# alexisvannson/GraphNet_Classifier

Hardware: AMD Instinct MI355X
Metric: edges aggregated/sec (GraphNet forward) (higher is better)
Workload: dtype f32; 1 GPU; c3: 1M nodes / 10M edges (6250 graphs x 160 nodes x 1600 edges), D=64, 2 GN blocks; graphs=6250, nodes=1000000, edges=10000000, n_blocks=2, width=64, step=CSR build + GraphNet.forward, inputs resident in HBM

## Files before the change

graphnet_classifier_amd/csrc/mlp_device.h:

```cpp
#pragma once
#include "gnc_common.h"

namespace gnc_mlp {

typedef float f32x16 __attribute__((ext_vector_type(16)));
typedef float f32x4 __attribute__((ext_vector_type(4)));

constexpr int KC = 64;
constexpr int LDSW = 68;
constexpr int RPW = 32;

__device__ __forceinline__ f32x16 mfma(float a, float b, f32x16 c) {
  return __builtin_amdgcn_mfma_f32_32x32x2f32(a, b, c, 0, 0, 0);
}

__device__ __forceinline__ void wave_lds_fence() {
  asm volatile("s_waitcnt lgkmcnt(0)" ::: "memory");
}

__device__ __forceinline__ float activate(float x, int act, float p) {
  switch (act) {
    case GNC_ACT_RELU: return x < 0.f ? 0.f : x;
    case GNC_ACT_IDENTITY: return x;
    case GNC_ACT_TANH: return tanhf(x);
// ... 933 lines not shown

struct BwdArgs {
  const float* grad_out;
  int ld_grad_out;
  float* act[GNC_MAX_LINEAR];
  float* dz[GNC_MAX_LINEAR];
  float* dx;
  int ld_dx;
  float* yhat;
  int dx_add_grad_out;
  float* ln_partial;
  const float* gg;
  const int* gg_index;
  int ld_gg;
  int64_t gg_rows;
  float* g_sum;
  int ld_g_sum;
};

__host__ __device__ inline int ldw_of(const gnc_mlp_desc_t& d, int l) { return d.ld_weight[l] ? d.ld_weight[l] : d.in_dim[l]; }

inline bool al16(const void* p) { return (reinterpret_cast<uintptr_t>(p) & 15u) == 0; }

inline int tiles_for(int width) {
  const int t = (width + 31) / 32;
  return t <= 1 ? 1 : t <= 2 ? 2 : t <= 4 ? 4 : 8;
}

int validate_desc(const gnc_mlp_desc_t* d, bool check_ptrs);
int launch_resident_dual(const float* x, int64_t ld_x, int64_t rows, const float* wa, int64_t ld_wa, const float* wb, int64_t ld_wb,
                         int in_dim, int out_dim, float* out_a, float* out_b, int64_t ld_out, hipStream_t stream, bool* launched);
int launch_resident(const gnc_mlp_desc_t& d, int T, bool narrow_out, hipStream_t stream, bool* launched,
                    bool probe_only = false, bool agg_only = false);
int launch_stream(const gnc_mlp_desc_t& d, int T, bool narrow_out, hipStream_t stream, bool* launched,
                  bool probe_only = false);
int launch_stream16(const gnc_mlp_desc_t& d, hipStream_t stream, bool* launched, bool probe_only = false);
int launch_col16(const gnc_mlp_desc_t& d, hipStream_t stream, bool* launched, bool probe_only = false);
int64_t col16_max_rows();
int64_t bwd_col16_max_rows();
bool bwd_col16_supported(const gnc_mlp_desc_t& d);
int bwd_col16_ln_partial_rows(int64_t rows);
int launch_bwd_col16(const gnc_mlp_bwd_desc_t& bd, hipStream_t stream);
bool bwd_col16_persist_supported(const gnc_mlp_desc_t& d);
int bwd_col16_persist_ln_partial_rows(int64_t rows);
int launch_bwd_col16_persist(const gnc_mlp_bwd_desc_t& bd, hipStream_t stream);
bool bwd_stream16_supported(const gnc_mlp_desc_t& d, bool want_dx);
int bwd_stream16_ln_partial_rows(int64_t rows);
int launch_bwd_stream16(const gnc_mlp_desc_t& d, const BwdArgs& b, hipStream_t stream, bool saved = false);

}
```

graphnet_classifier_amd/csrc/mlp_fused.hip:

```cpp
#include <stdlib.h>

#include "mlp_device.h"

using namespace gnc_mlp;

namespace {

constexpr int WAVES = 4;
constexpr int NT = WAVES * 64;
constexpr int RPB = RPW * WAVES;

__device__ __forceinline__ void stage_rows(float* abuf, const gnc_mlp_segment_t& seg, int64_t row0, int64_t rows,
                                           int c0, int ncol4, bool vec_ok, int lane) {
  const int c4 = lane & 15;
  const int rs = lane >> 4;
  if (c4 < ncol4) {
#pragma unroll
    for (int p = 0; p < RPW / 4; ++p) {
      const int j = p * 4 + rs;
      const int64_t r = row0 + j;
      f32x4 v = {0.f, 0.f, 0.f, 0.f};
      if (r < rows) {
        const int64_t tr = seg.index ? (int64_t)seg.index[r] : r;
        if (!seg.index || (uint64_t)tr < (uint64_t)seg.table_rows)
// ... 276 lines not shown
  if (rc) return rc;
  const auto [T, narrow_out] = tile_class(*desc);
  const gnc_mlp_desc_t probe = agg_probe(*desc);
  bool ok = false;
  {
    gnc_mlp_desc_t plain = *desc;
    plain.agg_out = nullptr;
    bool small = false;
    rc = launch_col16(plain, nullptr, &small, true);
    if (rc) return rc;
    if (small) {
      gnc::set_error("gnc_mlp_agg_supported: a small batch: run gnc_scatter_sum_csr_f32 on the output rows");
      return GNC_ERR_UNSUPPORTED;
    }
  }
  rc = launch_resident(probe, T, narrow_out, nullptr, &ok, true);
  if (rc) return rc;
  if (!ok && T == 4) {
    rc = launch_stream(probe, T, narrow_out, nullptr, &ok, true);
    if (rc) return rc;
  }
  if (!ok && T == 8) {
    rc = launch_stream16(probe, nullptr, &ok, true);
    if (rc) return rc;
  }
  if (!ok) {
    gnc::set_error("gnc_mlp_agg_supported: needs the weights-resident W-split shape (1 MATMUL + 2 ADD segments, residual = "
                   "the MATMUL segment, widths 33..64) or a 65..128-wide description of the streaming kernel");
    return GNC_ERR_UNSUPPORTED;
  }
  return GNC_OK;
}

extern "C" int gnc_mlp_agg_only_supported(const gnc_mlp_desc_t* desc) {
  int rc = gnc_mlp_agg_supported(desc);
  if (rc) return rc;
  const auto [T, narrow_out] = tile_class(*desc);
  const gnc_mlp_desc_t probe = agg_probe(*desc);
  bool ok = false;
  rc = launch_resident(probe, T, narrow_out, nullptr, &ok, true, true);
  if (rc) return rc;
  if (!ok) {
    gnc::set_error("gnc_mlp_agg_only_supported: needs the 64-wide W-split edge processor (1 MATMUL + 2 ADD segments, residual = "
                   "the MATMUL segment, three Linear layers, LayerNorm) without save_act");
    return GNC_ERR_UNSUPPORTED;
  }
  return GNC_OK;
}

extern "C" int gnc_mlp_forward_agg_only_f32(const gnc_mlp_desc_t* desc, void* stream) {
  int rc = validate_desc(desc, true);
  if (rc) return rc;
  if (!desc->agg_out || !desc->agg_index || !desc->agg_fix) {
    gnc::set_error("gnc_mlp_forward_agg_only_f32: agg_out, agg_index and agg_fix are required");
    return GNC_ERR_INVALID_ARGUMENT;
  }
  rc = gnc_mlp_agg_only_supported(desc);
  if (rc) return rc;
  if (desc->rows == 0) return GNC_OK;
  const auto [T, narrow_out] = tile_class(*desc);
  bool launched = false;
  rc = launch_resident(*desc, T, narrow_out, (hipStream_t)stream, &launched, false, true);
  if (!rc && !launched) {
    gnc::set_error("gnc_mlp_forward_agg_only_f32: the weights-resident kernel did not take the launch");
    rc = GNC_ERR_UNSUPPORTED;
  }
// ... 107 lines not shown
```

graphnet_classifier_amd/csrc/mlp_resident.hip:

```cpp
#include <stdlib.h>

#include "mlp_device.h"

using namespace gnc_mlp;

#ifdef GNC_PHASE_PROBE
__device__ unsigned long long gnc_phase_probe[4096 * 12];
extern "C" int gnc_phase_probe_read(void* dst, size_t bytes) {
  return (int)hipMemcpyFromSymbol(dst, HIP_SYMBOL(gnc_phase_probe), bytes);
}
#define PROBE_BEGIN() unsigned long long pr_acc[8] = {0, 0, 0, 0, 0, 0, 0, 0}, pr_tp, pr_tn; \
  const unsigned long long pr_c0 = __builtin_readcyclecounter(), pr_w0 = wall_clock64()
#define PROBE_TILE() pr_tp = __builtin_readcyclecounter()
#define PROBE(k) do { pr_tn = __builtin_readcyclecounter(); pr_acc[k] += pr_tn - pr_tp; pr_tp = pr_tn; } while (0)
#define PROBE_END() do { if ((threadIdx.x & 63) == 0) {                                                      \
    unsigned long long* o = gnc_phase_probe + (blockIdx.x * (blockDim.x >> 6) + (threadIdx.x >> 6)) * 12;    \
    for (int k = 0; k < 8; ++k) o[k] = pr_acc[k];                                                            \
    o[8] = __builtin_readcyclecounter() - pr_c0; o[9] = wall_clock64() - pr_w0; } } while (0)
#else
#define PROBE_BEGIN() do {} while (0)
#define PROBE_TILE() do {} while (0)
#define PROBE(k) do {} while (0)
#define PROBE_END() do {} while (0)
#endif

namespace {

constexpr int RWAVES = 8;
constexpr int RNT = RWAVES * 64;

template <int HT, int OT, int NMM, int NADD, bool RESREG, bool AGG = false, bool SAVE = false, bool FULL = false, int EF = 0, bool DUAL = false,
          int SPLIT = 0, bool AGGONLY = false>
__global__ __launch_bounds__(RNT) void mlp_resident_kernel(const gnc_mlp_desc_t d, const int num_wtiles,
                                                           const int total_chunks) {
  extern __shared__ __attribute__((aligned(16))) float lds[];
  constexpr int WT = HT > OT ? HT : OT;
  constexpr int CH = WT * 32 * LDSW;
  static_assert(!FULL || OT == 2, "fixed widths: 64 out");
  static_assert(!FULL || NADD == 2 || (NMM == 1 && !RESREG && !AGG && !SAVE && !DUAL), "fixed-width plain stacks");
  constexpr int SEGW = EF != 0 ? 3 : KC;
  constexpr bool W32 = FULL && !SAVE;
  constexpr bool GADD = W32 && NADD == 2;
  static_assert(SPLIT == 0 || (HT == 2 && SPLIT == 1 && NMM == 1 && ((NADD == 2 && RESREG && !DUAL) || (NADD == 0 && !RESREG))) ||
                    (HT == 2 && OT == 2 && SPLIT == 2 && NADD == 0 && !DUAL),
                "split shapes");
  constexpr int nf32 = SPLIT == 1 ? 0 : NMM;
  constexpr bool SPK = !(SPLIT == 1 && NADD == 2 && AGG && !FULL && !SAVE);
  constexpr bool PIPE = SPLIT != 0 && SPK && !DUAL && (FULL || (SPLIT == 2 && NMM == 1) || (SPLIT == 1 && NADD == 0));
  constexpr bool FRONT = GADD && SPLIT == 1 && PIPE;
  constexpr int GPK = FRONT ? 4 : 2;
  __bf16* const wsp = reinterpret_cast<__bf16*>(lds + nf32 * CH);
  auto wsplit = [&](int chunk) -> const __bf16* { return wsp + (chunk - nf32) * 3 * SPLANE; };
  constexpr int PSTRIDE = WT * 32;
  constexpr int NS = NMM + NADD;
  const int tid = threadIdx.x;
  const int lane = tid & 63;
  const int wave = __builtin_amdgcn_readfirstlane(tid >> 6);
  const int i = lane & 31;
  const int h = lane >> 5;
  const int c4 = lane & 15;
  const int rs = lane >> 4;
  const int L = FULL ? 3 : d.num_linear;
  const int out_dim = FULL ? KC : d.out_dim[L - 1];
  const int rows = (int)d.rows;
  float* wres = lds;
  float* pbuf = SPLIT == 0 ? lds + total_chunks * CH : lds + nf32 * CH + (total_chunks - nf32) * SCH;
  float* abuf = pbuf + (L + 2) * PSTRIDE + wave * RPW * LDSW;

  stage_params<RNT>(pbuf, d, PSTRIDE, tid);
  if constexpr (SPLIT != 0) {
    const int ldw0 = ldw_of(d, 0);
    const bool w0v = (ldw0 % 4 == 0) && ((reinterpret_cast<uintptr_t>(d.weight[0]) & 15u) == 0);
    if constexpr (SPLIT == 1) {
      stage_weights_split<RNT>(wsp, d.weight[0], ldw0, d.out_dim[0], d.seg[0].wcol, d.seg[0].wcol + d.seg[0].width,
                               w0v && (d.seg[0].wcol % 4 == 0), tid);
    } else {
#pragma unroll
      for (int s = 0; s < NMM; ++s)
        stage_weights<WT * 32, RNT>(wres + s * CH, d.weight[0], ldw0, d.out_dim[0], d.seg[s].wcol, d.seg[s].wcol + d.seg[s].width, 16,
                                    w0v && (d.seg[s].wcol % 4 == 0), tid);
// ... 54 lines not shown
    const int col = c4 * 4 < s.ld ? c4 * 4 : 0;
    if (s.index == nullptr) {
      if constexpr (W32)
        load_tile_rows_w(pre, table_window(s.ptr, rows, s.ld), s.ld, (wt < num_wtiles ? wt : num_wtiles) * RPW, rows, (uint32_t)(rs * s.ld + col) * 4u);
      else load_tile_rows(pre, s.ptr, s.ld, (int64_t)wt * RPW, rows, (uint32_t)(rs * s.ld + col) * 4u);
    } else {
      const __amdgpu_buffer_rsrc_t w = __builtin_amdgcn_make_buffer_rsrc(const_cast<float*>(s.ptr), 0, (int)s.bytes, 0x00020000);
      const uint32_t row_bytes = off * (uint32_t)(s.ld * 4);
#pragma unroll
      for (int p = 0; p < NP; ++p) pre[p] = window_load(w, (uint32_t)__shfl((int)row_bytes, p * 4 + rs, 64) + (uint32_t)(col * 4));
    }
  };
  auto stage = [&](const f32x4 (&pre)[NP], int width) {
    compiler_lds_barrier();
    const int c = c4 * 4;
    if (width >= KC) {
#pragma unroll
      for (int p = 0; p < NP; ++p) *reinterpret_cast<f32x4*>(abuf + (p * 4 + rs) * LDSW + c) = pre[p];
    } else {
#pragma unroll
      for (int p = 0; p < NP; ++p) {
        f32x4 v = pre[p];
        v.x = c + 0 < width ? v.x : 0.f; v.y = c + 1 < width ? v.y : 0.f;
        v.z = c + 2 < width ? v.z : 0.f; v.w = c + 3 < width ? v.w : 0.f;
        *reinterpret_cast<f32x4*>(abuf + (p * 4 + rs) * LDSW + c) = v;
      }
    }
    compiler_lds_barrier();
  };

  const int gwave = (int)blockIdx.x * RWAVES + wave;
  const int stride = AGG ? 1 : total_waves;
  int wt = gwave, wt_end = num_wtiles;
  if constexpr (AGG) {
    const int q = num_wtiles / total_waves, rem = num_wtiles - q * total_waves;
    wt = gwave * q + (gwave < rem ? gwave : rem);
    wt_end = wt + q + (gwave < rem ? 1 : 0);
  }
  f32x4 cur[NP];
  f32x4 addA[NADD ? NP : 1], addB[NADD ? NP : 1];
  uint32_t offs[NS];
  typedef float f32x2 __attribute__((ext_vector_type(2)));
  int ef_s = 0, ef_d = 0;
  f32x2 ef_ps = {0.f, 0.f}, ef_pd = {0.f, 0.f};
  const __amdgpu_buffer_rsrc_t ef_win =
      __builtin_amdgcn_make_buffer_rsrc(const_cast<float*>(EF == 1 ? d.ef_pos : nullptr), 0, EF == 1 ? (int)(uint32_t)(d.ef_nodes * 8) : 0, 0x00020000);
  auto ef_ids = [&](int t) {
    const int tc = t < last_wt ? t : last_wt;
    int r = tc * RPW + (lane & 31);
    r = r < rows ? r : rows - 1;
    ef_s = d.ef_src[r];
    ef_d = d.ef_dst[r];
  };
  auto ef_fetch = [&]() {
    typedef uint32_t u32x2 __attribute__((ext_vector_type(2)));
    ef_ps = __builtin_bit_cast(f32x2, (u32x2)__builtin_amdgcn_raw_buffer_load_b64(ef_win, (uint32_t)ef_s * 8u, 0, 0));
    ef_pd = __builtin_bit_cast(f32x2, (u32x2)__builtin_amdgcn_raw_buffer_load_b64(ef_win, (uint32_t)ef_d * 8u, 0, 0));
  };
  auto ef_stage = [&]() {
    compiler_lds_barrier();
    const float dx = ef_pd.x - ef_ps.x, dy = ef_pd.y - ef_ps.y;
    f32x4 v = {dx, dy, __builtin_fabsf(dx) + __builtin_fabsf(dy), 0.f};
    if (h) v = f32x4{0.f, 0.f, 0.f, 0.f};
    *reinterpret_cast<f32x4*>(abuf + i * LDSW + 4 * h) = v;
    compiler_lds_barrier();
  };
  typedef float f32x3 __attribute__((ext_vector_type(3)));
  f32x3 n3_row = {0.f, 0.f, 0.f};
  const __amdgpu_buffer_rsrc_t n3_win = __builtin_amdgcn_make_buffer_rsrc(
      const_cast<float*>(EF == 2 ? d.seg[0].ptr : nullptr), 0, EF == 2 ? (int)(uint32_t)(d.rows * 12) : 0, 0x00020000);
// ... 9 lines not shown
    *reinterpret_cast<f32x4*>(abuf + i * LDSW + 4 * h) = v;
    compiler_lds_barrier();
  };
  uint32_t off0 = 0;
  if constexpr (EF == 1) {
    ef_ids(wt);
    ef_fetch();
    ef_ids(wt + stride);
  } else if constexpr (EF == 2) {
    n3_fetch(wt);
  } else {
    load_rows(cur, sv[0], wt, row_offset(wt, sv[0]));
  }
#pragma unroll
  for (int s = 1; s < NS; ++s) offs[s] = row_offset(wt, sv[s]);
  if constexpr (EF == 0) off0 = row_offset(wt + stride, sv[0]);

  const int col_out = c4 * 4;
  const bool vec_out = FULL || ((out_dim % 4 == 0) && (d.ld_out % 4 == 0) && ((reinterpret_cast<uintptr_t>(d.out) & 15u) == 0));
  const uint32_t out_lane_off = (uint32_t)(rs * d.ld_out + col_out) * 4u;
  const uint32_t res_lane_off = (uint32_t)(rs * d.ld_residual + (col_out < d.ld_residual ? col_out : 0)) * 4u;

  auto agg_ids = [&](int t) -> int {
    int r = t * RPW + (lane & 31);
    r = r < rows ? r : rows - 1;
    return d.agg_index[r];
  };
  int aid = 0, aid_next = 0;
  float agg_acc = 0.f;
  int agg_cur = -1, agg_first_dst = -1;
  bool agg_first = true;
  if constexpr (AGG) aid = agg_ids(wt < last_wt ? wt : last_wt);
  static_assert(!AGGONLY || (AGG && FULL && !SAVE && !DUAL), "aggregate-only: the FULL AGG inference instance");
  int keep_lo = -1, keep_hi = -1;
  if constexpr (AGGONLY) {
    if (wt < wt_end) {
      const int last_row = wt_end * RPW < rows ? wt_end * RPW - 1 : rows - 1;
      keep_lo = d.agg_index[wt * RPW];
      keep_hi = d.agg_index[last_row];
    }
  }
  uint32_t keep_rows = 0;

  PROBE_BEGIN();
  while (wt < wt_end) {
    PROBE_TILE();
    const int row0 = wt * RPW;
    const int nwt = wt + stride;
    if constexpr (AGG) aid_next = agg_ids(nwt < last_wt ? nwt : last_wt);

    f32x16 hid[HT];
    f32x16 res[RESREG ? HT : 1];
    init_bias<HT>(hid, pbuf, h);
#pragma unroll
    for (int s = 0; s < NMM; ++s) {
      bool interleaved = false;
      if constexpr (EF == 1) ef_stage();
      else if constexpr (EF == 2) n3_stage();
      else stage(cur, sv[s].width);
      PROBE(0);
      if (s + 1 < NMM) {
        load_rows(cur, sv[s + 1 < NMM ? s + 1 : 0], wt, offs[s + 1 < NMM ? s + 1 : 0]);
        offs[s + 1 < NMM ? s + 1 : 0] = row_offset(nwt, sv[s + 1 < NMM ? s + 1 : 0]);
      } else {
        if constexpr (NADD > 0) {
          if (GADD || (sv[s].width == KC && sv[NMM].index && sv[NMM + 1].index)) {
            const SegView &sa = sv[NMM], &sb = sv[NMM + 1];
            const __amdgpu_buffer_rsrc_t wa = __builtin_amdgcn_make_buffer_rsrc(const_cast<float*>(sa.ptr), 0, (int)sa.bytes, 0x00020000);
            const __amdgpu_buffer_rsrc_t wb = __builtin_amdgcn_make_buffer_rsrc(const_cast<float*>(sb.ptr), 0, (int)sb.bytes, 0x00020000);
            const uint32_t cola = (uint32_t)(c4 * 4 < sa.ld ? c4 * 16 : 0), colb = (uint32_t)(c4 * 4 < sb.ld ? c4 * 16 : 0);
            const int rba = (int)(offs[NMM] * (uint32_t)(sa.ld * 4)), rbb = (int)(offs[NMM + 1] * (uint32_t)(sb.ld * 4));
            int na = __shfl(rba, rs, 64), nb = __shfl(rbb, rs, 64);
            if constexpr (SPLIT == 1) {
              const __bf16* wch = wsplit(s);
              auto request = [&](int kg) {
#pragma unroll
                for (int g = GPK * kg; g < GPK * kg + GPK && g < 8; ++g) {
                  const uint32_t oa = (uint32_t)na + cola, ob = (uint32_t)nb + colb;
                  if (g + 1 < 8) {
                    na = __shfl(rba, (g + 1) * 4 + rs, 64);
                    nb = __shfl(rbb, (g + 1) * 4 + rs, 64);
// ... 158 lines not shown
      f32x16 o[OT];
      init_bias<OT>(o, pbuf + (L - 1) * PSTRIDE, h);
      if constexpr (PIPE) mma_chunk_from_regs_split_pipe<HT, OT, 4>(o, hid, wsplit(NMM + L - 2), i, h);
      else if constexpr (SPLIT != 0) mma_chunk_from_regs_split<HT, OT, SPK>(o, hid, wsplit(NMM + L - 2), FULL ? KC : d.in_dim[L - 1], i, h);
      else mma_chunk_from_regs<HT, OT>(o, hid, wres + (NMM + L - 2) * CH, 0, FULL ? KC : d.in_dim[L - 1], i, h);
      PROBE(4);
      if (FULL || d.ln_gamma) layer_norm_tiles<OT>(o, pbuf + L * PSTRIDE, pbuf + (L + 1) * PSTRIDE, out_dim, d.ln_eps, h);
      if constexpr (RESREG) {
#pragma unroll
        for (int t = 0; t < OT && t < HT; ++t) o[t] += res[t < HT ? t : 0];
      }
      compiler_lds_barrier();
      tiles_to_lds<OT>(o, abuf, i, h);
      PROBE(5);
    }
    compiler_lds_barrier();
    if constexpr (AGG) {
      const int valid = rows - row0 < RPW ? rows - row0 : RPW;
      int prv = __shfl_up(aid, 1, 64);
      prv = lane == 0 ? agg_cur : prv;
      const unsigned long long vmask = valid >= 32 ? 0xffffffffull : ((1ull << valid) - 1ull);
      const unsigned long long bnd = __ballot(aid != prv) & vmask;
      if constexpr (AGGONLY) keep_rows = (uint32_t)(__ballot(aid == keep_lo || aid == keep_hi) & vmask);
      float rowv[RPW];
#pragma unroll
      for (int r = 0; r < RPW; ++r) rowv[r] = abuf[r * LDSW + lane];
      auto agg_row = [&](int r) {
        if ((bnd >> r) & 1ull) {
          if (agg_cur >= 0) {
            if (agg_first) {
              agg_first = false;
              agg_first_dst = agg_cur;
            } else if (lane < out_dim) {
              float* dstp = d.agg_out + (int64_t)agg_cur * d.ld_agg;
              asm volatile("s_nop 4\n\tglobal_store_dword %0, %1, %2\n\ts_nop 0" ::"v"(lane * 4), "v"(agg_acc), "s"(dstp) : "memory");
            }
          }
          agg_cur = __builtin_amdgcn_readlane(aid, r);
          agg_acc = 0.f;
        }
        agg_acc += rowv[r];
      };
#pragma unroll
      for (int r4 = 0; r4 < RPW; r4 += 4) {
        if (r4 + 4 <= valid && ((bnd >> r4) & 0xfull) == 0) {
          agg_acc += rowv[r4 + 0];
          agg_acc += rowv[r4 + 1];
          agg_acc += rowv[r4 + 2];
          agg_acc += rowv[r4 + 3];
        } else {
#pragma unroll
          for (int r = r4; r < r4 + 4; ++r)
            if (r < valid) agg_row(r);
        }
      }
      aid = aid_next;
    }
    if constexpr (EF == 1) {
      asm volatile("" ::"v"(ef_ps), "v"(ef_pd), "v"(ef_s), "v"(ef_d));
    } else if constexpr (EF == 2) {
      asm volatile("" ::"v"(n3_row.x), "v"(n3_row.y), "v"(n3_row.z));
    } else {
#pragma unroll
      for (int p = 0; p < NP; ++p) asm volatile("" ::"v"(cur[p]));
    }
#pragma unroll
    for (int s = 1; s < NS; ++s) asm volatile("" ::"v"(offs[s]));
    asm volatile("" ::"v"(off0));
    if constexpr (AGG) asm volatile("" ::"v"(aid_next));

    if constexpr (AGGONLY) {
      if (keep_rows) {
#pragma unroll
        for (int p = 0; p < NP; ++p) {
          const f32x4 v = *reinterpret_cast<const f32x4*>(abuf + (p * 4 + rs) * LDSW + col_out);
          if ((keep_rows >> (p * 4 + rs)) & 1u)
            hidden_window_store<true>(v, out_lane_off + (uint32_t)(row0 + 4 * p) * (uint32_t)(d.ld_out * 4), table_window(d.out, rows, d.ld_out));
        }
      }
    } else {
      f32x4 outv[NP];
#pragma unroll
      for (int p = 0; p < NP; ++p) outv[p] = *reinterpret_cast<const f32x4*>(abuf + (p * 4 + rs) * LDSW + col_out);
      if ((!FULL || NADD != 0) && !RESREG && d.residual) {
        f32x4 rv[NP];
        load_tile_rows(rv, d.residual, d.ld_residual, row0, rows, res_lane_off);
#pragma unroll
        for (int p = 0; p < NP; ++p) outv[p] += rv[p];
      }
      if constexpr (W32) {
        store_tile_rows_w<true>(outv, table_window(d.out, rows, d.ld_out), d.ld_out, row0, rows, out_lane_off);
      } else if (vec_out) {
        if (col_out < out_dim) {
          if (row0 + RPW <= rows) {
            uint32_t r0b;
            const __amdgpu_buffer_rsrc_t ow = full_tile_window(d.out, row0, rows, d.ld_out, &r0b);
#pragma unroll
            for (int p = 0; p < NP; ++p) hidden_window_store_s<true>(outv[p], out_lane_off + r0b, ow, (uint32_t)(p * 16 * d.ld_out));
          } else {
#pragma unroll
            for (int p = 0; p < NP; ++p) hidden_window_store(outv[p], out_lane_off, row_window(d.out, row0 + 4 * p, rows, d.ld_out));
          }
        }
      } else {
#pragma unroll
        for (int p = 0; p < NP; ++p) {
          const int r = row0 + p * 4 + rs;
          store_row_piece(d.out + (int64_t)(r < rows ? r : rows - 1) * d.ld_out, col_out, outv[p], r < rows && col_out < out_dim,
                          out_dim, false);
        }
      }
    }
    if constexpr (DUAL) {
      compiler_lds_barrier();
      tiles_to_lds<HT>(hidb, abuf, i, h);
      compiler_lds_barrier();
      f32x4 outb[NP];
#pragma unroll
      for (int p = 0; p < NP; ++p) outb[p] = *reinterpret_cast<const f32x4*>(abuf + (p * 4 + rs) * LDSW + col_out);
      if (col_out < out_dim) {
        if (row0 + RPW <= rows) {
          uint32_t r0b;
          const __amdgpu_buffer_rsrc_t ow = full_tile_window(d.save_act[0], row0, rows, d.ld_out, &r0b);
#pragma unroll
          for (int p = 0; p < NP; ++p) hidden_window_store_s<true>(outb[p], out_lane_off + r0b, ow, (uint32_t)(p * 16 * d.ld_out));
        } else {
#pragma unroll
          for (int p = 0; p < NP; ++p) hidden_window_store(outb[p], out_lane_off, row_window(d.save_act[0], row0 + 4 * p, rows, d.ld_out));
        }
      }
    }
    compiler_lds_barrier();
    PROBE(6);
    wt = nwt;
  }
  if constexpr (AGG) {
    if (lane == 0) {
      d.agg_fix[2 * gwave] = agg_first ? agg_cur : agg_first_dst;
      d.agg_fix[2 * gwave + 1] = agg_cur;
    }
  }
  PROBE_END();
}

template <int HT, int OT, int NMM, int NADD, bool RESREG, bool AGG = false, bool SAVE = false, bool FULL = false, int EF = 0, bool DUAL = false,
          int SPLIT = 0, bool AGGONLY = false>
int launch(const gnc_mlp_desc_t& d, int total_chunks, size_t smem, hipStream_t stream) {
  void (*const kernel)(const gnc_mlp_desc_t, const int, const int) = &mlp_resident_kernel<HT, OT, NMM, NADD, RESREG, AGG, SAVE, FULL, EF, DUAL, SPLIT, AGGONLY>;
  static bool attr_set = false;
  if (!attr_set) {
    int rc = gnc::check_hip(hipFuncSetAttribute(reinterpret_cast<const void*>(kernel), hipFuncAttributeMaxDynamicSharedMemorySize, 160 * 1024),
                            "hipFuncSetAttribute(MaxDynamicSharedMemorySize)");
    if (rc) return rc;
    attr_set = true;
  }
  const int64_t num_wtiles = gnc::ceil_div(d.rows, RPW);
  int64_t grid = gnc::ceil_div(num_wtiles, RWAVES);
  if (grid > gnc::num_cu()) grid = gnc::num_cu();
  if constexpr (AGG) grid = gnc::num_cu();
  kernel<<<dim3((unsigned)grid), dim3(RNT), smem, stream>>>(d, (int)num_wtiles, total_chunks);
  return gnc::check_launch("mlp_resident_kernel");
}

template <int HT, int OT, int NMM, int NADD, bool RESREG, bool AGG = false, bool SAVE = false, bool FULL = false, int EF = 0,
          bool AGGONLY = false>
int launch_cls(int split, const gnc_mlp_desc_t& d, int total_chunks, size_t smem, hipStream_t stream) {
  if constexpr (HT == 2 && OT == 2 && NMM == 1 && NADD == 2 && RESREG) {
    if (split == 1) return launch<HT, OT, NMM, NADD, RESREG, AGG, SAVE, FULL, EF, false, 1, AGGONLY>(d, total_chunks, smem, stream);
  }
  if constexpr (HT == 2 && NMM == 1 && NADD == 0 && !RESREG && !AGG && !SAVE && !FULL && EF == 0) {
    if (split == 1) return launch<HT, OT, NMM, NADD, RESREG, AGG, SAVE, FULL, EF, false, 1>(d, total_chunks, smem, stream);
  }
  if constexpr (HT == 2 && OT == 2 && NADD == 0 && !AGG && (!FULL || EF != 0) && ((NMM == 1 && !RESREG) || (NMM == 2 && EF == 0))) {
    if (split == 2) return launch<HT, OT, NMM, NADD, RESREG, AGG, SAVE, FULL, EF, false, 2>(d, total_chunks, smem, stream);
  }
  if (split) return GNC_ERR_UNSUPPORTED;
  return launch<HT, OT, NMM, NADD, RESREG, AGG, SAVE, FULL, EF, false, 0, AGGONLY>(d, total_chunks, smem, stream);
}

}

static bool f32_exact() {
  static const bool v = getenv("GNC_MLP_F32_EXACT") != nullptr;
  return v;
}

extern "C" int gnc_mlp_agg_fix_len(void) { return 2 * gnc::num_cu() * RWAVES; }

int gnc_mlp::launch_resident_dual(const float* x, int64_t ld_x, int64_t rows, const float* wa, int64_t ld_wa, const float* wb,
                                  int64_t ld_wb, int in_dim, int out_dim, float* out_a, float* out_b, int64_t ld_out,
                                  hipStream_t stream, bool* launched) {
  *launched = false;
  static const bool disabled = getenv("GNC_MLP_NO_RESIDENT") != nullptr;
  if (disabled || rows < 1 || rows >= INT32_MAX || in_dim < 1 || in_dim > KC || out_dim <= 32 || out_dim > KC || out_dim % 4 != 0 ||
      ld_x % 4 != 0 || ld_x < in_dim || ld_out % 4 != 0 || ld_out < out_dim || ld_wa < in_dim || ld_wb < in_dim || ld_wa > INT32_MAX ||
      ld_wb > INT32_MAX || ld_x > INT32_MAX || ld_out > INT32_MAX || !al16(x) || !al16(out_a) || !al16(out_b))
    return GNC_OK;
  gnc_mlp_desc_t d = {};
  d.num_segments = 1;
  d.num_linear = 1;
  d.activation = GNC_ACT_RELU;
  d.seg[0].ptr = x;
  d.seg[0].width = in_dim;
  d.seg[0].ld = (int32_t)ld_x;
  d.seg[0].mode = GNC_SEG_MATMUL;
  d.weight[0] = wa;
  d.ld_weight[0] = (int32_t)ld_wa;
  d.weight[1] = wb;
  d.ld_weight[1] = (int32_t)ld_wb;
  d.in_dim[0] = in_dim;
  d.out_dim[0] = out_dim;
  d.in_dim[1] = in_dim;
  d.out = out_a;
  d.save_act[0] = out_b;
  d.ld_out = (int32_t)ld_out;
  d.rows = rows;
  const int total_chunks = 2;
  const bool split = !f32_exact();
  const size_t floats = (size_t)total_chunks * (split ? SCH : 2 * 32 * LDSW) + (size_t)(1 + 2) * 2 * 32 + (size_t)RWAVES * RPW * LDSW;
  *launched = true;
// ... 162 lines not shown
```

graphnet_classifier_amd/native.py:

```python
from __future__ import annotations

import ctypes
import math
import os
from ctypes import POINTER, Structure, c_char_p, c_double, c_float, c_int32, c_int64, c_size_t, c_void_p

import torch

LIB_NAME = "libgnc_hip.so"
LIB_PATH = os.path.join(os.path.dirname(os.path.abspath(__file__)), LIB_NAME)

GNC_MAX_SEGMENTS = 4
GNC_MAX_LINEAR = 8
ABI_VERSION = 20

ACTIVATIONS = {
    "ReLU": 0, "Identity": 1, "Tanh": 2, "Sigmoid": 3, "SiLU": 4, "GELU": 5, "LeakyReLU": 6, "ELU": 7,
}

_SIGNATURES = {
    "gnc_abi_version": (c_int32, []),
    "gnc_last_error_string": (c_char_p, []),
    "gnc_target_arch": (c_char_p, []),
    "gnc_mlp_agg_supported": (c_int32, [c_void_p]),
    "gnc_mlp_agg_only_supported": (c_int32, [c_void_p]),
    "gnc_mlp_forward_agg_only_f32": (c_int32, [c_void_p, c_void_p]),
    "gnc_mlp_edge_features_supported": (c_int32, [c_void_p]),
    "gnc_mlp_operands_in_place_supported": (c_int32, [c_void_p]),
    "gnc_mlp_save_act_supported": (c_int32, [c_void_p]),
    "gnc_mlp_agg_fix_len": (c_int32, []),
    "gnc_mlp_small_batch_supported": (c_int32, [c_void_p]),
    "gnc_mlp_small_batch_max_rows": (c_int64, []),
    "gnc_mlp_projection_t2_f32": (c_int32, [c_void_p, c_int64, c_void_p, c_int64, c_int64, c_void_p, c_int64, c_int32, c_int32, c_void_p,
                                            c_int64, c_void_p]),
    "gnc_mlp_dual_projection_f32": (c_int32, [c_void_p, c_int64, c_int64, c_void_p, c_int64, c_void_p, c_int64, c_int32, c_int32,
                                              c_void_p, c_void_p, c_int64, c_void_p]),
    "gnc_mlp_backward_small_batch_supported": (c_int32, [c_void_p]),
    "gnc_readout_forward_f32": (c_int32, [c_void_p, c_int64, c_void_p, c_int64, c_void_p, c_int32, c_void_p, c_int64, c_void_p, c_int32,
                                          c_void_p, c_int64, c_void_p, c_int32, c_void_p, c_void_p, c_void_p, c_void_p, c_void_p]),
    "gnc_readout_backward_f32": (c_int32, [c_void_p, c_void_p, c_int64, c_void_p, c_int64, c_int32, c_void_p, c_int64, c_int32, c_void_p,
                                           c_int64, c_int32, c_void_p, c_void_p, c_void_p, c_void_p, c_void_p, c_void_p, c_void_p, c_void_p,
                                           c_void_p, c_void_p]),
    "gnc_readout_batched_supported": (c_int32, [c_int64, c_int64, c_int32, c_int32, c_int32, c_void_p]),
    "gnc_readout_batched_forward_f32": (c_int32, [c_void_p, c_void_p, c_int64, c_int64, c_int32, c_int64, c_void_p, c_int64, c_void_p,
                                                  c_int32, c_void_p, c_int64, c_void_p, c_int32, c_void_p, c_int64, c_void_p, c_int32,
                                                  c_void_p, c_void_p, c_void_p, c_void_p, c_int64, c_void_p]),
    "gnc_readout_batched_backward_f32": (c_int32, [c_void_p, c_void_p, c_void_p, c_int64, c_int64, c_int32, c_int64, c_void_p, c_int64,
                                                   c_int32, c_void_p, c_int64, c_int32, c_void_p, c_int64, c_int32, c_void_p, c_void_p,
                                                   c_void_p, c_void_p, c_void_p, c_void_p, c_int64, c_void_p]),
    "gnc_pad_graph_batch_supported": (c_int32, [c_int64, c_int64, c_int64, c_int64, c_int64, c_int32, c_int32]),
    "gnc_pad_graph_batch": (c_int32, [c_void_p, c_int32, c_void_p, c_int32, c_void_p, c_int64, c_int64, c_int64, c_int64, c_void_p, c_void_p,
                                      c_void_p, c_int64, c_int64, c_void_p, c_void_p, c_void_p, c_void_p, c_void_p, c_void_p, c_void_p]),
    "gnc_xty_small_max_rows": (c_int32, []),
    "gnc_xty_small_f32": (c_int32, [c_void_p, c_int32, c_void_p]),
    "gnc_agg_fixup_f32": (c_int32, [c_void_p, c_int64, c_void_p, c_void_p, c_int32, c_int64, c_int32, c_void_p, c_int64,
                                    c_void_p]),
    "gnc_csr_workspace_bytes": (c_size_t, [c_int64, c_int64]),
    "gnc_csr_build": (c_int32, [c_void_p, c_int64, c_int64, c_void_p, c_void_p, c_void_p, c_void_p, c_size_t, c_void_p]),
    "gnc_topology_workspace_bytes": (c_size_t, [c_int64, c_int64, c_int32]),
    "gnc_topology_build": (c_int32, [c_void_p, c_void_p, c_int32, c_int64, c_int64, c_void_p, c_void_p, c_void_p, c_void_p, c_void_p,
                                     c_void_p, c_size_t, c_int32, c_void_p]),
    "gnc_permute_index_i64_i32": (c_int32, [c_void_p, c_void_p, c_int64, c_void_p, c_void_p]),
    "gnc_permute_index_checked_i64_i32": (c_int32, [c_void_p, c_void_p, c_int64, c_int64, c_void_p, c_void_p, c_void_p]),
# ... 677 lines not shown
    return _saved_act_honoured(lib, desc, [any_tensor.data_ptr()] * (desc.num_linear - 1), need_dx, fused)


def mlp_forward(segments, weights, biases, ln=None, activation: str = "ReLU", act_param: float = 0.0,
                residual: torch.Tensor | None = None, rows: int | None = None, modes=None, aggregate=None,
                save_act: list | None = None, save_need_dx: bool = True, agg_only: bool = False):
    lib = load_library()
    given = (segments, weights, biases, residual, rows, modes)
    small = _rows_of(segments, rows) <= _small_batch_rows(lib)
    raw = not small and save_act is None and aggregate is None
    segs, weights, biases, residual, rows, modes = _prepare_mlp(*given, vector_rows=not (small or raw))
    dev = segs[0][0].device
    out = torch.empty(rows, weights[-1].size(0), dtype=torch.float32, device=dev)
    desc = make_mlp_desc(segs, weights, biases, ln, activation, act_param, residual, out, rows)
    if raw and any(t.data_ptr() % 16 or _ld(t) % 4 for t in [sg[0] for sg in segs] + weights) and \
            lib.gnc_mlp_operands_in_place_supported(ctypes.byref(desc)) != 0:
        segs, weights, biases, residual, rows, modes = _prepare_mlp(*given)
        desc = make_mlp_desc(segs, weights, biases, ln, activation, act_param, residual, out, rows)
    if small and lib.gnc_mlp_small_batch_supported(ctypes.byref(desc)) != 0:
        segs, weights, biases, residual, rows, modes = _prepare_mlp(*given)
        desc = make_mlp_desc(segs, weights, biases, ln, activation, act_param, residual, out, rows)
    if (save_act is not None and SAVE_ACT and rows > 0 and len(weights) >= 2
            and lib.gnc_mlp_save_act_supported(ctypes.byref(desc)) == 0 and _backward_reads_saved_act(lib, desc, out, save_need_dx)):
        for l in range(len(weights) - 1):
            a = torch.empty(rows, weights[l].size(0), dtype=torch.float32, device=dev)
            desc.save_act[l] = a.data_ptr()
            save_act.append(a)
    agg = fix = None
    if aggregate is not None:
        dst_of_row, rowptr, num_nodes = aggregate
        _require_cuda(dst_of_row, rowptr)
        if rows > 0 and lib.gnc_mlp_agg_supported(ctypes.byref(desc)) == 0:
            agg = torch.empty(num_nodes, out.size(1), dtype=torch.float32, device=dev)
            fix = torch.empty(lib.gnc_mlp_agg_fix_len(), dtype=torch.int32, device=dev)
            desc.agg_out, desc.ld_agg = agg.data_ptr(), _ld(agg)
            desc.agg_index, desc.agg_fix = dst_of_row.contiguous().data_ptr(), fix.data_ptr()
    agg_only = agg_only and agg is not None and lib.gnc_mlp_agg_only_supported(ctypes.byref(desc)) == 0
    forward = lib.gnc_mlp_forward_agg_only_f32 if agg_only else lib.gnc_mlp_forward_f32
    flops = 2.0 * rows * sum(w.size(0) * w.size(1) for w in weights)
    with torch.cuda.device(dev):
        nadd = sum(1 for m in modes if m == SEG_ADD)
        _check(_launch(f"mlp_fused_in{weights[0].size(1)}{'+%dadd' % nadd if nadd else ''}_h{weights[0].size(0)}"
                       f"_out{weights[-1].size(0)}_L{len(weights)}", out,
                       lambda: forward(ctypes.byref(desc), _stream(out)), flops),
               forward.__name__)
        if agg is not None:
            _check(lib.gnc_agg_fixup_f32(out.data_ptr(), _ld(out), rowptr.data_ptr(), fix.data_ptr(), fix.numel(), num_nodes,
                                         out.size(1), agg.data_ptr(), _ld(agg), _stream(out)), "gnc_agg_fixup_f32")
    return (None if agg_only else out, agg) if aggregate is not None else out


FOLD_EDGE_FEATURES = os.environ.get("GNC_NO_K6_FOLD") is None


def mlp_forward_edge_features(pos: torch.Tensor, src: torch.Tensor, dst: torch.Tensor, weights, biases, ln=None,
                              activation: str = "ReLU", act_param: float = 0.0):
    lib = load_library()
    if not FOLD_EDGE_FEATURES or pos.dim() != 2 or pos.size(1) != 2 or src.numel() == 0:
        return None
    _require_cuda(pos, src, dst)
    if src.dtype != torch.int32 or dst.dtype != torch.int32:
        raise TypeError("edge endpoint ids must be int32")
    pos = pos.float().contiguous()
    src, dst = src.contiguous(), dst.contiguous()
    rows, sd = src.numel(), pos.size(1)
    if weights[0].size(1) != sd + 1 or rows <= _small_batch_rows(lib):
        return None
    weights = [_rowmajor(w.detach()) for w in weights]
    biases = [b.contiguous() if b is not None else None for b in biases]
    dev = pos.device
    out = torch.empty(rows, weights[-1].size(0), dtype=torch.float32, device=dev)
    desc = make_mlp_desc([(pos, None, sd + 1, SEG_MATMUL, 0)], weights, biases, ln, activation, act_param, None, out, rows)
    desc.seg[0].ld = 4
    desc.ef_pos, desc.ef_src, desc.ef_dst = pos.data_ptr(), src.data_ptr(), dst.data_ptr()
    desc.ef_nodes, desc.ef_space_dim = pos.size(0), sd
    if lib.gnc_mlp_edge_features_supported(ctypes.byref(desc)) != 0:
        return None
    flops = 2.0 * rows * sum(w.size(0) * w.size(1) for w in weights)
    with torch.cuda.device(dev):
        _check(_launch(f"mlp_fused_in{weights[0].size(1)}_h{weights[0].size(0)}_out{weights[-1].size(0)}_L{len(weights)}", out,
# ... 1038 lines not shown
```

include/gnc_hip.h:

```cpp
#ifndef GNC_HIP_H
#define GNC_HIP_H

#include <stddef.h>
#include <stdint.h>

#ifdef __cplusplus
extern "C" {
#endif

#define GNC_ABI_VERSION 20

enum {
  GNC_OK = 0,
  GNC_ERR_INVALID_ARGUMENT = -1,
  GNC_ERR_UNSUPPORTED = -2,
  GNC_ERR_WORKSPACE = -3,
  GNC_ERR_HIP = -4
};

#define GNC_MAX_SEGMENTS 4
#define GNC_MAX_LINEAR 8

enum { GNC_ACT_RELU = 0, GNC_ACT_IDENTITY = 1, GNC_ACT_TANH = 2, GNC_ACT_SIGMOID = 3,
       GNC_ACT_SILU = 4, GNC_ACT_GELU = 5, GNC_ACT_LEAKY_RELU = 6, GNC_ACT_ELU = 7 };
// ... 49 lines not shown
  int32_t activation;
  float act_param;
  gnc_mlp_segment_t seg[GNC_MAX_SEGMENTS];
  const float* weight[GNC_MAX_LINEAR];
  int32_t ld_weight[GNC_MAX_LINEAR];
  const float* bias[GNC_MAX_LINEAR];
  int32_t in_dim[GNC_MAX_LINEAR];
  int32_t out_dim[GNC_MAX_LINEAR];
  const float* ln_gamma;
  const float* ln_beta;
  float ln_eps;
  const float* residual;
  int32_t ld_residual;
  float* out;
  int32_t ld_out;
  int64_t rows;
  float* agg_out;
  int32_t ld_agg;
  const int32_t* agg_index;
  int32_t* agg_fix;
  float* save_act[GNC_MAX_LINEAR];
  const float* ef_pos;
  const int32_t* ef_src;
  const int32_t* ef_dst;
  int64_t ef_nodes;
  int32_t ef_space_dim;
} gnc_mlp_desc_t;

size_t gnc_sizeof_mlp_desc(void);
int gnc_mlp_supported(const gnc_mlp_desc_t* desc );
int gnc_mlp_forward_f32(const gnc_mlp_desc_t* desc , void* stream);
int gnc_mlp_agg_supported(const gnc_mlp_desc_t* desc );
int gnc_mlp_agg_fix_len(void);
int gnc_mlp_agg_only_supported(const gnc_mlp_desc_t* desc );
int gnc_mlp_forward_agg_only_f32(const gnc_mlp_desc_t* desc , void* stream);
int gnc_mlp_operands_in_place_supported(const gnc_mlp_desc_t* desc );
int gnc_mlp_edge_features_supported(const gnc_mlp_desc_t* desc );
int gnc_mlp_small_batch_supported(const gnc_mlp_desc_t* desc );
int gnc_mlp_projection_t2_f32(const float* a, int64_t ld_a, const float* b, int64_t ld_b, int64_t rows, const float* w, int64_t ld_w,
                              int32_t hidden, int32_t dn, float* out, int64_t ld_out, void* stream);
int64_t gnc_mlp_small_batch_max_rows(void);
int gnc_mlp_dual_projection_f32(const float* x, int64_t ld_x, int64_t rows, const float* wa, int64_t ld_wa, const float* wb,
                                int64_t ld_wb, int32_t in_dim, int32_t out_dim, float* out_a, float* out_b, int64_t ld_out,
                                void* stream);
int gnc_mlp_save_act_supported(const gnc_mlp_desc_t* desc );
int gnc_agg_fixup_f32(const float* src, int64_t ld_src, const int32_t* rowptr, const int32_t* fix, int32_t n_fix,
                      int64_t num_nodes, int32_t feat_dim, float* out, int64_t ld_out, void* stream);

typedef struct gnc_mlp_bwd_desc {
  gnc_mlp_desc_t fwd;
  const float* grad_out;
  int32_t ld_grad_out;
  float* act[GNC_MAX_LINEAR];
  float* dz[GNC_MAX_LINEAR];
  float* dx;
  int32_t ld_dx;
  float* yhat;
  int32_t dx_add_grad_out;
  float* ln_partial;
  float* dw_partial[GNC_MAX_LINEAR];
  const float* grad_gather;
  int32_t ld_grad_gather;
  const int32_t* grad_gather_index;
  int64_t grad_gather_rows;
  float* grad_sum;
  int32_t ld_grad_sum;
// ... 223 lines not shown
```

Before: 3.607 billion edges/s.

## Dynamically schedule aggregating edge tiles in runs via atomic counters

Replaces the static contiguous split of edge tiles across waves in the aggregating resident kernel with fixed-length runs handed out by atomic counters, spread over eight counters keyed by block index. Each run emits its own boundary fix-up entry, so the fix array grows to one entry per run. A small prepare kernel resets the unused fix slots and seeds the counters. The goal is to balance load across waves and shrink tail imbalance, at the cost of an extra launch, atomics, and more fix-up work.

```diff
diff --git a/graphnet_classifier_amd/csrc/mlp_device.h b/graphnet_classifier_amd/csrc/mlp_device.h
--- a/graphnet_classifier_amd/csrc/mlp_device.h
+++ b/graphnet_classifier_amd/csrc/mlp_device.h
@@ -989,6 +989,7 @@
                          int in_dim, int out_dim, float* out_a, float* out_b, int64_t ld_out, hipStream_t stream, bool* launched);
 int launch_resident(const gnc_mlp_desc_t& d, int T, bool narrow_out, hipStream_t stream, bool* launched,
                     bool probe_only = false, bool agg_only = false);
+int resident_agg_fix_entries(int64_t rows);
 int launch_stream(const gnc_mlp_desc_t& d, int T, bool narrow_out, hipStream_t stream, bool* launched,
                   bool probe_only = false);
 int launch_stream16(const gnc_mlp_desc_t& d, hipStream_t stream, bool* launched, bool probe_only = false);
diff --git a/graphnet_classifier_amd/csrc/mlp_fused.hip b/graphnet_classifier_amd/csrc/mlp_fused.hip
--- a/graphnet_classifier_amd/csrc/mlp_fused.hip
+++ b/graphnet_classifier_amd/csrc/mlp_fused.hip
@@ -332,6 +332,15 @@
   return GNC_OK;
 }
 
+extern "C" int gnc_mlp_agg_fix_len_for(const gnc_mlp_desc_t* desc) {
+  if (validate_desc(desc, false)) return gnc_mlp_agg_fix_len();
+  const auto [T, narrow_out] = tile_class(*desc);
+  const gnc_mlp_desc_t probe = agg_probe(*desc);
+  bool resident = false;
+  if (launch_resident(probe, T, narrow_out, nullptr, &resident, true) || !resident) return gnc_mlp_agg_fix_len();
+  return resident_agg_fix_entries(desc->rows);
+}
+
 extern "C" int gnc_mlp_agg_only_supported(const gnc_mlp_desc_t* desc) {
   int rc = gnc_mlp_agg_supported(desc);
   if (rc) return rc;
diff --git a/graphnet_classifier_amd/csrc/mlp_resident.hip b/graphnet_classifier_amd/csrc/mlp_resident.hip
--- a/graphnet_classifier_amd/csrc/mlp_resident.hip
+++ b/graphnet_classifier_amd/csrc/mlp_resident.hip
@@ -32,7 +32,7 @@
 template <int HT, int OT, int NMM, int NADD, bool RESREG, bool AGG = false, bool SAVE = false, bool FULL = false, int EF = 0, bool DUAL = false,
           int SPLIT = 0, bool AGGONLY = false>
 __global__ __launch_bounds__(RNT) void mlp_resident_kernel(const gnc_mlp_desc_t d, const int num_wtiles,
-                                                           const int total_chunks) {
+                                                           const int total_chunks, const int agg_run, int32_t* const agg_cnt) {
   extern __shared__ __attribute__((aligned(16))) float lds[];
   constexpr int WT = HT > OT ? HT : OT;
   constexpr int CH = WT * 32 * LDSW;
@@ -46,6 +46,7 @@
                 "split shapes");
   constexpr int nf32 = SPLIT == 1 ? 0 : NMM;
   constexpr bool SPK = !(SPLIT == 1 && NADD == 2 && AGG && !FULL && !SAVE);
+  constexpr bool RUNS = AGG && SPK;
   constexpr bool PIPE = SPLIT != 0 && SPK && !DUAL && (FULL || (SPLIT == 2 && NMM == 1) || (SPLIT == 1 && NADD == 0));
   constexpr bool FRONT = GADD && SPLIT == 1 && PIPE;
   constexpr int GPK = FRONT ? 4 : 2;
@@ -166,10 +167,39 @@
   const int gwave = (int)blockIdx.x * RWAVES + wave;
   const int stride = AGG ? 1 : total_waves;
   int wt = gwave, wt_end = num_wtiles;
+  int run_end = num_wtiles, run_slot = gwave, nrun = num_wtiles, nnrun = num_wtiles, part_end = 0;
+  int32_t* run_cnt = nullptr;
+  int tick = 0;
+  bool run_first_tile = true;
+  auto run_take = [&]() {
+    if (lane == 0) tick = (int)atomicInc(reinterpret_cast<unsigned int*>(run_cnt), 0xffffffffu);
+  };
+  auto run_tile = [&]() -> int {
+    const int r = __builtin_amdgcn_readfirstlane(tick);
+    return r < part_end ? r * agg_run : num_wtiles;
+  };
   if constexpr (AGG) {
-    const int q = num_wtiles / total_waves, rem = num_wtiles - q * total_waves;
-    wt = gwave * q + (gwave < rem ? gwave : rem);
-    wt_end = wt + q + (gwave < rem ? 1 : 0);
+    if (RUNS && agg_run > 0) {
+      const int grid = (int)gridDim.x, label = (int)blockIdx.x & 7, per = grid >> 3, extra = grid & 7;
+      const int64_t num_runs = (num_wtiles + agg_run - 1) / agg_run;
+      const int before = (label + 1) * per + (label + 1 < extra ? label + 1 : extra);
+      part_end = (int)(num_runs * before / grid);
+      run_cnt = agg_cnt + label;
+      run_take();
+      wt = run_tile();
+      if (wt < num_wtiles) {
+        run_take();
+        nrun = run_tile();
+      }
+      wt_end = wt + agg_run < num_wtiles ? wt + agg_run : num_wtiles;
+      run_slot = wt / agg_run;
+    } else {
+      const int q = num_wtiles / total_waves, rem = num_wtiles - q * total_waves;
+      wt = gwave * q + (gwave < rem ? gwave : rem);
+      wt_end = wt + q + (gwave < rem ? 1 : 0);
+      if (wt >= wt_end) wt = num_wtiles;
+    }
+    run_end = wt_end;
   }
   f32x4 cur[NP];
   f32x4 addA[NADD ? NP : 1], addB[NADD ? NP : 1];
@@ -245,21 +275,44 @@
   bool agg_first = true;
   if constexpr (AGG) aid = agg_ids(wt < last_wt ? wt : last_wt);
   static_assert(!AGGONLY || (AGG && FULL && !SAVE && !DUAL), "aggregate-only: the FULL AGG inference instance");
-  int keep_lo = -1, keep_hi = -1;
+  auto fix_out = [&](int slot, int first_dst, int last_dst) {
+    int32_t* const p = d.agg_fix + 2 * (int64_t)slot;
+    const int v = lane == 0 ? first_dst : last_dst;
+    if (lane < 2) asm volatile("s_nop 4\n\tglobal_store_dword %0, %1, %2\n\ts_nop 0" ::"v"(lane * 4), "v"(v), "s"(p) : "memory");
+  };
+  int keep_lo = -1, keep_hi = -1, nkeep_lo = -1, nkeep_hi = -1;
+  auto run_last_row = [&](int first_tile) -> int {
+    const int e = first_tile + agg_run < num_wtiles ? first_tile + agg_run : num_wtiles;
+    return e * RPW < rows ? e * RPW - 1 : rows - 1;
+  };
   if constexpr (AGGONLY) {
-    if (wt < wt_end) {
-      const int last_row = wt_end * RPW < rows ? wt_end * RPW - 1 : rows - 1;
+    if (wt < num_wtiles) {
+      const int last_row = run_end * RPW < rows ? run_end * RPW - 1 : rows - 1;
       keep_lo = d.agg_index[wt * RPW];
       keep_hi = d.agg_index[last_row];
     }
   }
   uint32_t keep_rows = 0;
+  auto run_ahead = [&]() {
+    run_take();
+    if constexpr (AGGONLY) {
+      nkeep_lo = d.agg_index[nrun * RPW];
+      nkeep_hi = d.agg_index[run_last_row(nrun)];
+    }
+  };
+  if constexpr (AGG) {
+    if (RUNS && nrun < num_wtiles) run_ahead();
+#pragma unroll
+    for (int p = 0; p < NP; ++p) asm volatile("" ::"v"(cur[p]));
+    if (RUNS && agg_run == 0 && wt >= num_wtiles) fix_out(run_slot, -1, -1);
+  }
 
   PROBE_BEGIN();
-  while (wt < wt_end) {
+  while (wt < (AGG ? num_wtiles : wt_end)) {
     PROBE_TILE();
     const int row0 = wt * RPW;
-    const int nwt = wt + stride;
+    const bool run_last_tile = AGG && wt + 1 >= run_end;
+    const int nwt = AGG ? (run_last_tile ? nrun : wt + 1) : wt + stride;
     if constexpr (AGG) aid_next = agg_ids(nwt < last_wt ? nwt : last_wt);
 
     f32x16 hid[HT];
@@ -484,7 +537,7 @@
               agg_first = false;
               agg_first_dst = agg_cur;
             } else if (lane < out_dim) {
-              float* dstp = d.agg_out + (int64_t)agg_cur * d.ld_agg;
+              float* dstp = d.agg_out + (int64_t)__builtin_amdgcn_readfirstlane(agg_cur) * d.ld_agg;
               asm volatile("s_nop 4\n\tglobal_store_dword %0, %1, %2\n\ts_nop 0" ::"v"(lane * 4), "v"(agg_acc), "s"(dstp) : "memory");
             }
           }
@@ -520,6 +573,30 @@
     for (int s = 1; s < NS; ++s) asm volatile("" ::"v"(offs[s]));
     asm volatile("" ::"v"(off0));
     if constexpr (AGG) asm volatile("" ::"v"(aid_next));
+    if constexpr (AGG) {
+      if constexpr (RUNS) asm volatile("" ::"v"(tick));
+      if constexpr (AGGONLY) asm volatile("" ::"v"(nkeep_lo), "v"(nkeep_hi));
+      if (RUNS && run_first_tile && nrun < num_wtiles) nnrun = run_tile();
+      run_first_tile = false;
+      if (RUNS && run_last_tile) {
+        fix_out(run_slot, agg_first ? agg_cur : agg_first_dst, agg_cur);
+        agg_cur = -1;
+        agg_first_dst = -1;
+        agg_first = true;
+        run_first_tile = true;
+        if (RUNS && nrun < num_wtiles) {
+          run_slot = nrun / agg_run;
+          run_end = nrun + agg_run < num_wtiles ? nrun + agg_run : num_wtiles;
+        }
+        nrun = nnrun;
+        nnrun = num_wtiles;
+        if constexpr (AGGONLY) {
+          keep_lo = __builtin_amdgcn_readfirstlane(nkeep_lo);
+          keep_hi = __builtin_amdgcn_readfirstlane(nkeep_hi);
+        }
+        if (RUNS && nrun < num_wtiles) run_ahead();
+      }
+    }
 
     if constexpr (AGGONLY) {
       if (keep_rows) {
@@ -586,19 +663,53 @@
     PROBE(6);
     wt = nwt;
   }
-  if constexpr (AGG) {
-    if (lane == 0) {
-      d.agg_fix[2 * gwave] = agg_first ? agg_cur : agg_first_dst;
-      d.agg_fix[2 * gwave + 1] = agg_cur;
-    }
-  }
+  if constexpr (AGG && !RUNS) fix_out(run_slot, agg_first ? agg_cur : agg_first_dst, agg_cur);
   PROBE_END();
+}
+
+constexpr int kAggCounters = 8;
+constexpr int kAggRunMin = 12, kAggRunMax = 24;
+int agg_run_forced() {
+  const char* e = getenv("GNC_AGG_RUN_TILES");
+  if (!e || !*e) return 0;
+  const long v = strtol(e, nullptr, 10);
+  return v < 1 ? 1 : v > (1 << 20) ? (1 << 20) : (int)v;
+}
+int agg_run_tiles(int64_t rows) {
+  const int64_t num_wtiles = gnc::ceil_div(rows, RPW), waves = (int64_t)gnc::num_cu() * RWAVES;
+  const int forced = agg_run_forced();
+  if (forced) return (int64_t)forced * waves >= num_wtiles ? 0 : forced;
+  int best = 0;
+  int64_t best_depth = 0;
+  for (int r = kAggRunMin; r <= kAggRunMax && (int64_t)r * waves < num_wtiles; ++r) {
+    const int64_t depth = gnc::ceil_div(gnc::ceil_div(num_wtiles, r), waves) * r;
+    if (!best || depth <= best_depth) best = r, best_depth = depth;
+  }
+  if (best && best_depth * waves * 50 > num_wtiles * 51) best = 0;
+  return best;
+}
+int agg_fix_entries(int64_t rows) {
+  const int r = agg_run_tiles(rows);
+  const int64_t per_wave = 2 * (int64_t)gnc::num_cu() * RWAVES;
+  const int64_t per_run = r ? 2 * gnc::ceil_div(gnc::ceil_div(rows, RPW), r) : 0;
+  return (int)(per_run > per_wave ? per_run : per_wave);
+}
+
+__global__ void mlp_agg_prepare_kernel(int32_t* fix, int from, int to, int32_t* cnt, int64_t num_runs, int grid) {
+  const int j = from + (int)(blockIdx.x * blockDim.x + threadIdx.x);
+  if (j < to) fix[j] = -1;
+  if (blockIdx.x == 0 && threadIdx.x < kAggCounters) {
+    const int label = (int)threadIdx.x, per = grid >> 3, extra = grid & 7;
+    const int before = label * per + (label < extra ? label : extra);
+    cnt[label] = (int32_t)(num_runs * before / grid);
+  }
 }
 
 template <int HT, int OT, int NMM, int NADD, bool RESREG, bool AGG = false, bool SAVE = false, bool FULL = false, int EF = 0, bool DUAL = false,
           int SPLIT = 0, bool AGGONLY = false>
 int launch(const gnc_mlp_desc_t& d, int total_chunks, size_t smem, hipStream_t stream) {
-  void (*const kernel)(const gnc_mlp_desc_t, const int, const int) = &mlp_resident_kernel<HT, OT, NMM, NADD, RESREG, AGG, SAVE, FULL, EF, DUAL, SPLIT, AGGONLY>;
+  void (*const kernel)(const gnc_mlp_desc_t, const int, const int, const int, int32_t* const) =
+      &mlp_resident_kernel<HT, OT, NMM, NADD, RESREG, AGG, SAVE, FULL, EF, DUAL, SPLIT, AGGONLY>;
   static bool attr_set = false;
   if (!attr_set) {
     int rc = gnc::check_hip(hipFuncSetAttribute(reinterpret_cast<const void*>(kernel), hipFuncAttributeMaxDynamicSharedMemorySize, 160 * 1024),
@@ -610,7 +721,27 @@
   int64_t grid = gnc::ceil_div(num_wtiles, RWAVES);
   if (grid > gnc::num_cu()) grid = gnc::num_cu();
   if constexpr (AGG) grid = gnc::num_cu();
-  kernel<<<dim3((unsigned)grid), dim3(RNT), smem, stream>>>(d, (int)num_wtiles, total_chunks);
+  int agg_run = 0;
+  int32_t* agg_cnt = nullptr;
+  if constexpr (AGG) {
+    agg_run = agg_run_tiles(d.rows);
+    if (agg_run) {
+      const int n_fix = agg_fix_entries(d.rows);
+      const int64_t num_runs = gnc::ceil_div(num_wtiles, agg_run);
+      agg_cnt = d.agg_fix + n_fix;
+      constexpr bool runs = !(SPLIT == 1 && NADD == 2 && !FULL && !SAVE);
+      int from = (int)(2 * num_runs);
+      if constexpr (!runs) {
+        agg_run = 0;
+        from = 2 * (int)grid * RWAVES;
+      }
+      const int blocks = (int)gnc::ceil_div((int64_t)(n_fix - from > 0 ? n_fix - from : 1), 256);
+      mlp_agg_prepare_kernel<<<dim3(blocks), dim3(256), 0, stream>>>(d.agg_fix, from, n_fix, agg_cnt, num_runs, (int)grid);
+      int rc = gnc::check_launch("mlp_agg_prepare_kernel");
+      if (rc) return rc;
+    }
+  }
+  kernel<<<dim3((unsigned)grid), dim3(RNT), smem, stream>>>(d, (int)num_wtiles, total_chunks, agg_run, agg_cnt);
   return gnc::check_launch("mlp_resident_kernel");
 }
 
@@ -638,6 +769,9 @@
 }
 
 extern "C" int gnc_mlp_agg_fix_len(void) { return 2 * gnc::num_cu() * RWAVES; }
+extern "C" int gnc_mlp_agg_counter_len(void) { return kAggCounters; }
+extern "C" int gnc_mlp_agg_run_tiles(int64_t rows) { return agg_run_tiles(rows < 0 ? 0 : rows); }
+int gnc_mlp::resident_agg_fix_entries(int64_t rows) { return agg_fix_entries(rows < 0 ? 0 : rows); }
 
 int gnc_mlp::launch_resident_dual(const float* x, int64_t ld_x, int64_t rows, const float* wa, int64_t ld_wa, const float* wb,
                                   int64_t ld_wb, int in_dim, int out_dim, float* out_a, float* out_b, int64_t ld_out,
diff --git a/graphnet_classifier_amd/native.py b/graphnet_classifier_amd/native.py
--- a/graphnet_classifier_amd/native.py
+++ b/graphnet_classifier_amd/native.py
@@ -29,6 +29,9 @@
     "gnc_mlp_operands_in_place_supported": (c_int32, [c_void_p]),
     "gnc_mlp_save_act_supported": (c_int32, [c_void_p]),
     "gnc_mlp_agg_fix_len": (c_int32, []),
+    "gnc_mlp_agg_fix_len_for": (c_int32, [c_void_p]),
+    "gnc_mlp_agg_counter_len": (c_int32, []),
+    "gnc_mlp_agg_run_tiles": (c_int32, [c_int64]),
     "gnc_mlp_small_batch_supported": (c_int32, [c_void_p]),
     "gnc_mlp_small_batch_max_rows": (c_int64, []),
     "gnc_mlp_projection_t2_f32": (c_int32, [c_void_p, c_int64, c_void_p, c_int64, c_int64, c_void_p, c_int64, c_int32, c_int32, c_void_p,
@@ -772,7 +775,8 @@
         _require_cuda(dst_of_row, rowptr)
         if rows > 0 and lib.gnc_mlp_agg_supported(ctypes.byref(desc)) == 0:
             agg = torch.empty(num_nodes, out.size(1), dtype=torch.float32, device=dev)
-            fix = torch.empty(lib.gnc_mlp_agg_fix_len(), dtype=torch.int32, device=dev)
+            n_fix = lib.gnc_mlp_agg_fix_len_for(ctypes.byref(desc))
+            fix = torch.empty(n_fix + lib.gnc_mlp_agg_counter_len(), dtype=torch.int32, device=dev)
             desc.agg_out, desc.ld_agg = agg.data_ptr(), _ld(agg)
             desc.agg_index, desc.agg_fix = dst_of_row.contiguous().data_ptr(), fix.data_ptr()
     agg_only = agg_only and agg is not None and lib.gnc_mlp_agg_only_supported(ctypes.byref(desc)) == 0
@@ -785,7 +789,7 @@
                        lambda: forward(ctypes.byref(desc), _stream(out)), flops),
                forward.__name__)
         if agg is not None:
-            _check(lib.gnc_agg_fixup_f32(out.data_ptr(), _ld(out), rowptr.data_ptr(), fix.data_ptr(), fix.numel(), num_nodes,
+            _check(lib.gnc_agg_fixup_f32(out.data_ptr(), _ld(out), rowptr.data_ptr(), fix.data_ptr(), n_fix, num_nodes,
                                          out.size(1), agg.data_ptr(), _ld(agg), _stream(out)), "gnc_agg_fixup_f32")
     return (None if agg_only else out, agg) if aggregate is not None else out
 
diff --git a/include/gnc_hip.h b/include/gnc_hip.h
--- a/include/gnc_hip.h
+++ b/include/gnc_hip.h
@@ -105,6 +105,9 @@
 int gnc_mlp_forward_f32(const gnc_mlp_desc_t* desc , void* stream);
 int gnc_mlp_agg_supported(const gnc_mlp_desc_t* desc );
 int gnc_mlp_agg_fix_len(void);
+int gnc_mlp_agg_fix_len_for(const gnc_mlp_desc_t* desc );
+int gnc_mlp_agg_counter_len(void);
+int gnc_mlp_agg_run_tiles(int64_t rows);
 int gnc_mlp_agg_only_supported(const gnc_mlp_desc_t* desc );
 int gnc_mlp_forward_agg_only_f32(const gnc_mlp_desc_t* desc , void* stream);
 int gnc_mlp_operands_in_place_supported(const gnc_mlp_desc_t* desc );
```

After: 3.634 billion edges/s, median of 6. No clear change (+0.7%).
